# YuePanEdward/MULLS

Measured on AMD Instinct MI355X. Metric: scan-pair registrations/sec (64-beam ~120k pts, 20 ICP iters); dT vs ref, higher is better.
Workload: dtype f32

## Files before the change

mulls_amd/csrc/k_reduce.hip:

```cpp
#include "device_util.h"
#include "accum.h"
#include "solve_wave.h"

template <int LANES, int MIN_WG>
__global__ __launch_bounds__(LANES, MIN_WG) void k_accum(const uint32_t *__restrict__ leaders, const Job *__restrict__ jobs, const CloudDesc *__restrict__ descs,
														 const PairState *__restrict__ states, RunParams rp, const float4 *__restrict__ spos,
														 const float4 *__restrict__ mq, const uint8_t *__restrict__ flag, float *__restrict__ wd,
														 double *__restrict__ partial)
{
	extern __shared__ __attribute__((aligned(16))) unsigned char lds_raw[];
	__shared__ double part[MULLS_NTERM_PAD];
	const uint32_t job_idx = leaders[xcd_job(blockIdx.x, gridDim.x)];
	const Job job = jobs[job_idx];
	const PairState &ps = states[job.pair];
	if (!ps.active && !ps.want_residual)
		return;
	const CloudDesc *pd = descs + job.pair * MULLS_NC;
	const bool residual_pass = ps.want_residual != 0;
	int cnt[MULLS_NC];
	for (int c = 0; c < MULLS_NC; c++)
		cnt[c] = (int)(class_called(rp, pd[c], c) ? pd[c].valid_next : pd[c].n_valid);
	const AccumCtx A = accum_ctx(rp, job.cls, ps.iter, residual_pass, class_weight(rp, job.cls, residual_pass, cnt));
	trip_sum<true, LANES>(A, ps.x, pd[job.cls], job.start, spos, mq, flag, wd, lds_raw, part);
	if (threadIdx.x < MULLS_NTERM)
		partial[(size_t)job_idx * MULLS_NTERM + threadIdx.x] = part[threadIdx.x];
}

namespace
{
template <typename TS, int W0, int WIN, int MODE, int METRIC, int A0>
__device__ __forceinline__ void add_window(const AccumCtx &A, const double *x, const float4 P, const float4 Q, const float4 N, float wi, float &w, double *acc, const float *wpre)
{
	TS t[WIN];
#pragma unroll
	for (int k = 0; k < WIN; k++)
		t[k] = (TS)0;
	point_terms<TS, W0, WIN, MODE, METRIC>(A, x, P, Q, N, wi, w, t, wpre);
#pragma unroll
	for (int k = 0; k < WIN; k++)
		acc[W0 - A0 + k] += (double)t[k];
}
#ifndef MULLS_ACCW_WIN
#define MULLS_ACCW_WIN 9
#endif
#ifndef MULLS_ACCW_WIN_D
#define MULLS_ACCW_WIN_D 12
#endif
template <typename TS, int W0, int REM, int MODE, int METRIC, int A0>
__device__ __forceinline__ void add_windows(const AccumCtx &A, const double *x, const float4 P, const float4 Q, const float4 N, float wi, float &w, double *acc, const float *wpre)
{
	constexpr int WMAX = sizeof(TS) == 8 ? MULLS_ACCW_WIN_D : MULLS_ACCW_WIN;
	constexpr int WIN = REM < WMAX ? REM : WMAX;
	add_window<TS, W0, WIN, MODE, METRIC, A0>(A, x, P, Q, N, wi, w, acc, wpre);
	if constexpr (REM > WIN)
		add_windows<TS, W0 + WIN, REM - WIN, MODE, METRIC, A0>(A, x, P, Q, N, wi, w, acc, wpre);
}
template <typename TS, int NT, int MODE, int METRIC, int T0, int NTW>
__device__ __forceinline__ void wave_trip(const AccumCtx &A, const double *x, const CloudDesc &d, uint32_t trip0, const float4 *__restrict__ spos, const float4 *__restrict__ mq,
										   const uint8_t *__restrict__ flag, float *__restrict__ wd, double *__restrict__ out, bool owner, const LiveWord *__restrict__ live,
										   uint32_t cloud)
{
	const uint32_t lane = threadIdx.x & 63u;
	const uint32_t src_n = d.src_n, src_off = d.src_off;
	const uint32_t n_here = min(src_n - trip0, (uint32_t)MULLS_ACC_LANES), iters = (n_here + 63u) >> 6;
	const bool compacted = d.compacted != 0u;
	const uint32_t last = src_off + (compacted ? max(d.src_c, 1u) : src_n) - 1u;
	const unsigned long long below_me = (1ull << lane) - 1ull;
	static_assert(MULLS_ACC_LANES / 64 <= 64, "one LiveWord per lane covers a trip");
	uint32_t lw_lo = 0u, lw_hi = 0u, lw_below = 0u;
	if (compacted)
	{
		const LiveWord w = live[live_word_base(d, cloud) + (trip0 >> 6) + min(lane, iters - 1u)];
		lw_lo = (uint32_t)w.alive, lw_hi = (uint32_t)(w.alive >> 32), lw_below = w.below;
	}
	struct Rec
	{
		uint32_t f, g;
		bool live;
		float4 P, Q;
		float3 N;
		float w;
	};
	const bool need_w = A.residual_pass, writes_w = !A.residual_pass && (METRIC != 2 || !A.faithful);
	auto load = [&](uint32_t i) {
		Rec r;
		uint32_t g = src_off + trip0 + lane + 64u * i;
		r.live = true;
		if (compacted)
		{
			const unsigned long long alive = ((unsigned long long)(uint32_t)__builtin_amdgcn_readlane((int)lw_hi, (int)i) << 32) | (uint32_t)__builtin_amdgcn_readlane((int)lw_lo, (int)i);
			g = src_off + (uint32_t)__builtin_amdgcn_readlane((int)lw_below, (int)i) + (uint32_t)__popcll(alive & below_me);
			r.live = ((alive >> lane) & 1ull) != 0ull;
		}
		g = min(g, last);
		r.g = g;
		r.f = flag[g];
		r.P = spos[g], r.Q = mq[2u * g], r.N = *reinterpret_cast<const float3 *>(mq + 2u * g + 1u);
		r.w = need_w ? wd[g] : 0.0f;
		return r;
	};
	double acc[NTW];
#pragma unroll
	for (int k = 0; k < NTW; k++)
		acc[k] = -0.0;
#define MULLS_PIN_REC(r) asm volatile("" : "+v"((r).f), "+v"((r).P.x), "+v"((r).Q.x), "+v"((r).N.x), "+v"((r).w))
#if MULLS_ACCW_PREFETCH
	Rec cur = load(0);
#endif
	for (uint32_t i = 0; i < iters; i++)
	{
#if MULLS_ACCW_PREFETCH
		MULLS_PIN_REC(cur);
		Rec nxt = cur;
		if (i + 1u < iters)
			nxt = load(i + 1u);
#else
		Rec cur = load(i);
		MULLS_PIN_REC(cur);
#endif
		const uint32_t s = trip0 + lane + 64u * i;
		const bool valid = s < src_n && cur.live && (cur.f & (MULLS_F_ALIVE | MULLS_F_VALID)) == (MULLS_F_ALIVE | MULLS_F_VALID);
		if (valid)
		{
			float w = cur.w;
			const float4 N4 = make_float4(cur.N.x, cur.N.y, cur.N.z, 0.0f);
			const float wi = (A.inten_w && !A.residual_pass) ? point_wi(cur.P, cur.Q) : 1.0f;
			const float wpre = A.residual_pass ? 0.0f : corr_weight(A, METRIC, cur.P, cur.Q, N4, wi);
			add_windows<TS, T0, NTW, MODE, METRIC, T0>(A, x, cur.P, cur.Q, N4, wi, w, acc, A.residual_pass ? nullptr : &wpre);
			if (owner && writes_w)
				wd[cur.g] = w;
		}
#if MULLS_ACCW_PREFETCH
		cur = nxt;
#endif
	}
	if (NTW == NT && lane < MULLS_NTERM)
	{
		const bool has = MODE == 1 ? li_slot((int)lane) >= 0 : (int)lane < NT;
		if (!has)
			out[lane] = 0.0;
	}
#pragma unroll
	for (int k = 0; k < NTW; k++)
	{
		double sum = acc[k];
		sum = dpp_add_f64<0xB1>(sum);
		sum = dpp_add_f64<0x4E>(sum);
		sum = dpp_add_f64<0x141>(sum);
		sum = dpp_add_f64<0x140>(sum);
		sum = dpp_add_f64_rows<0x142, 0xa>(sum);
		sum = dpp_add_f64_rows<0x143, 0xc>(sum);
		acc[k] = sum;
	}
	if (lane == 63u)
	{
#pragma unroll
		for (int k = 0; k < NTW; k++)
			out[MODE == 1 ? li_term(T0 + k) : T0 + k] = acc[k];
	}
}
}

#ifndef MULLS_ACCW_SPLIT
#define MULLS_ACCW_SPLIT 1
#endif
#ifndef MULLS_ACCW_PREFETCH
#define MULLS_ACCW_PREFETCH 0
#endif
#ifndef MULLS_ACCW_OCC
#define MULLS_ACCW_OCC 4
#endif
#define MULLS_ACCW_WAVES 4
__global__ __launch_bounds__(64 * MULLS_ACCW_WAVES, MULLS_ACCW_OCC) void k_accum_wave(const uint32_t *__restrict__ leaders, uint32_t n_trips, const Job *__restrict__ jobs,
																					   const CloudDesc *__restrict__ descs, const PairState *__restrict__ states, RunParams rp,
																					   const float4 *__restrict__ spos, const float4 *__restrict__ mq, const uint8_t *__restrict__ flag,
																					   float *__restrict__ wd, double *__restrict__ partial)
{
	const uint32_t wave = threadIdx.x >> 6, part = wave % MULLS_ACCW_SPLIT;
	const uint32_t trip = blockIdx.x * (MULLS_ACCW_WAVES / MULLS_ACCW_SPLIT) + wave / MULLS_ACCW_SPLIT;
	if (trip >= n_trips)
		return;
	const uint32_t job_idx = leaders[trip];
	const Job job = jobs[job_idx];
	const PairState &ps = states[job.pair];
	if (!ps.active && !ps.want_residual)
		return;
	const CloudDesc *pd = descs + job.pair * MULLS_NC;
	const bool residual_pass = ps.want_residual != 0;
	int cnt[MULLS_NC];
	for (int c = 0; c < MULLS_NC; c++)
		cnt[c] = (int)(class_called(rp, pd[c], c) ? pd[c].valid_next : pd[c].n_valid);
	const AccumCtx A = accum_ctx(rp, job.cls, ps.iter, residual_pass, class_weight(rp, job.cls, residual_pass, cnt));
	const CloudDesc &d = pd[job.cls];
	const uint32_t ci = job.pair * MULLS_NC + job.cls;
	double *out = partial + (size_t)job_idx * MULLS_NTERM;
	if (d.src_n <= job.start)
	{
		if (part == 0u && (threadIdx.x & 63u) < MULLS_NTERM)
			out[threadIdx.x & 63u] = 0.0;
		return;
	}
	if (residual_pass || A.metric == 1)
	{
		if (part)
			return;
		if (!residual_pass)
			wave_trip<double, 12, 1, 1, 0, 12>(A, ps.x, d, job.start, spos, mq, flag, wd, out, true, rp.live_mask, ci);
		else if (A.metric == 0)
			wave_trip<double, 2, 0, 0, 0, 2>(A, ps.x, d, job.start, spos, mq, flag, wd, out, true, rp.live_mask, ci);
		else if (A.metric == 1)
			wave_trip<double, 2, 0, 1, 0, 2>(A, ps.x, d, job.start, spos, mq, flag, wd, out, true, rp.live_mask, ci);
		else
			wave_trip<double, 2, 0, 2, 0, 2>(A, ps.x, d, job.start, spos, mq, flag, wd, out, true, rp.live_mask, ci);
	}
#if MULLS_ACCW_SPLIT == 2
	else if (A.metric == 0)
	{
		if (part == 0u)
			wave_trip<float, 27, 0, 0, 0, 14>(A, ps.x, d, job.start, spos, mq, flag, wd, out, true, rp.live_mask, ci);
		else
			wave_trip<float, 27, 0, 0, 14, 13>(A, ps.x, d, job.start, spos, mq, flag, wd, out, false, rp.live_mask, ci);
	}
	else
	{
		if (part == 0u)
			wave_trip<float, 27, 0, 2, 0, 14>(A, ps.x, d, job.start, spos, mq, flag, wd, out, true, rp.live_mask, ci);
		else
			wave_trip<float, 27, 0, 2, 14, 13>(A, ps.x, d, job.start, spos, mq, flag, wd, out, false, rp.live_mask, ci);
	}
#else
	else if (A.metric == 0)
		wave_trip<float, 27, 0, 0, 0, 27>(A, ps.x, d, job.start, spos, mq, flag, wd, out, true, rp.live_mask, ci);
	else
		wave_trip<float, 27, 0, 2, 0, 27>(A, ps.x, d, job.start, spos, mq, flag, wd, out, true, rp.live_mask, ci);
#endif
}

namespace
{
struct FinishLds
{
	double sums[MULLS_NC][MULLS_NTERM_PAD], comb[MULLS_NTERM_PAD];
	uint32_t cnt[32];
};
__device__ __forceinline__ void finish_pair(CloudDesc *pd, const PairState &ps, const RunParams &rp, const double *__restrict__ partial,
											 PairOut &o, const uint32_t *__restrict__ pair_bbox, FinishLds *M = nullptr)
{
	if (threadIdx.x >= 192 && threadIdx.x < 198)
	{
		const uint32_t v = pair_bbox[threadIdx.x - 192];
		o.bbox[threadIdx.x - 192] = v;
		if (M)
			M->cnt[24 + threadIdx.x - 192] = v;
	}
	if (threadIdx.x < MULLS_NC * MULLS_NTERM)
	{
		const int c = threadIdx.x / MULLS_NTERM, t = threadIdx.x % MULLS_NTERM;
		if (rp.used[c])
		{
			constexpr uint32_t STEP = MULLS_ACC_LANES / MULLS_SRC_PER_BLOCK;
			double sum = 0.0;
			uint32_t j = pd[c].job_begin;
			const uint32_t je = pd[c].job_end;
			for (; j + 32u * STEP <= je; j += 32u * STEP)
			{
				double v[32];
#pragma unroll
				for (uint32_t k = 0; k < 32u; k++)
					v[k] = partial[(size_t)(j + k * STEP) * MULLS_NTERM + t];
#pragma unroll
				for (uint32_t k = 0; k < 32u; k++)
					sum += v[k];
			}
			for (; j + 16u * STEP <= je; j += 16u * STEP)
			{
				double v[16];
#pragma unroll
				for (uint32_t k = 0; k < 16u; k++)
					v[k] = partial[(size_t)(j + k * STEP) * MULLS_NTERM + t];
#pragma unroll
				for (uint32_t k = 0; k < 16u; k++)
					sum += v[k];
			}
			for (; j < je; j += STEP)
				sum += partial[(size_t)j * MULLS_NTERM + t];
			o.sums[c][t] = sum;
			if (M)
				M->sums[c][t] = sum;
		}
	}
	__syncthreads();
	if (rp.pull_comb && threadIdx.x >= 64 && threadIdx.x < 64 + MULLS_NTERM)
	{
		if (M)
		{
			combine_rows(rp, ps.want_residual != 0, M->sums, M->comb, (int)threadIdx.x - 64);
			o.comb[threadIdx.x - 64] = M->comb[threadIdx.x - 64];
		}
		else
			combine_rows(rp, ps.want_residual != 0, o.sums, o.comb, (int)threadIdx.x - 64);
	}
	if (threadIdx.x < MULLS_NC)
	{
		const int c = threadIdx.x;
		CloudDesc &d = pd[c];
		if (ps.active)
		{
			if (class_called(rp, d, c))
			{
				d.n_valid = d.valid_next;
				d.alive_cur = d.alive_next;
			}
			d.alive_next = 0;
			d.valid_next = 0;
			d.n_matched = 0;
		}
		o.n_valid[c] = d.n_valid;
		o.n_alive[c] = d.alive_cur;
		o.src_n[c] = d.src_n;
		o.tgt_n[c] = d.tgt_n;
		if (M)
			M->cnt[c] = d.n_valid, M->cnt[6 + c] = d.alive_cur, M->cnt[12 + c] = d.src_n, M->cnt[18 + c] = d.tgt_n;
	}
}
__device__ __forceinline__ void finish_pair_wave(CloudDesc *pd, const PairState &ps, const RunParams &rp, const double *__restrict__ partial, PairOut &o,
												  const uint32_t *__restrict__ pair_bbox, FinishLds &M)
{
	const uint32_t l = threadIdx.x;
	constexpr uint32_t STEP = MULLS_ACC_LANES / MULLS_SRC_PER_BLOCK;
	if (l >= 32u && l < 38u)
	{
		const uint32_t v = pair_bbox[l - 32u];
		o.bbox[l - 32u] = v;
		M.cnt[24u + l - 32u] = v;
	}
	double sum[3] = {0.0, 0.0, 0.0};
	uint32_t j[3], je[3];
	bool on[3];
#pragma unroll
	for (int u = 0; u < 3; u++)
	{
		const uint32_t idx = l + 64u * (uint32_t)u, c = idx / MULLS_NTERM;
		on[u] = idx < MULLS_NC * MULLS_NTERM && rp.used[c < MULLS_NC ? c : 0u];
		j[u] = on[u] ? pd[c].job_begin : 0u;
		je[u] = on[u] ? pd[c].job_end : 0u;
	}
	double v[3][4];
#pragma unroll
	for (int u = 0; u < 3; u++)
	{
		const uint32_t t = (l + 64u * (uint32_t)u) % MULLS_NTERM;
#pragma unroll
		for (uint32_t k = 0; k < 4u; k++)
			v[u][k] = j[u] + k * STEP < je[u] ? partial[(size_t)(j[u] + k * STEP) * MULLS_NTERM + t] : 0.0;
	}
#pragma unroll
	for (int u = 0; u < 3; u++)
	{
		const uint32_t idx = l + 64u * (uint32_t)u, c = idx / MULLS_NTERM, t = idx % MULLS_NTERM;
#pragma unroll
		for (uint32_t k = 0; k < 4u; k++)
			if (j[u] + k * STEP < je[u])
				sum[u] += v[u][k];
		for (uint32_t jj = j[u] + 4u * STEP; jj < je[u]; jj += STEP)
			sum[u] += partial[(size_t)jj * MULLS_NTERM + t];
		if (on[u])
		{
			o.sums[c][t] = sum[u];
			M.sums[c][t] = sum[u];
		}
	}
	__syncthreads();
	if (rp.pull_comb && l < MULLS_NTERM)
	{
		combine_rows(rp, ps.want_residual != 0, M.sums, M.comb, (int)l);
		o.comb[l] = M.comb[l];
	}
	if (l >= 56u && l < 56u + MULLS_NC)
	{
		const int c = (int)l - 56;
		CloudDesc &d = pd[c];
		if (ps.active)
		{
			if (class_called(rp, d, c))
			{
				d.n_valid = d.valid_next;
				d.alive_cur = d.alive_next;
			}
			d.alive_next = 0;
			d.valid_next = 0;
			d.n_matched = 0;
		}
		o.n_valid[c] = d.n_valid;
		o.n_alive[c] = d.alive_cur;
		o.src_n[c] = d.src_n;
		o.tgt_n[c] = d.tgt_n;
		M.cnt[c] = d.n_valid, M.cnt[6 + c] = d.alive_cur, M.cnt[12 + c] = d.src_n, M.cnt[18 + c] = d.tgt_n;
	}
}
}

__global__ __launch_bounds__(MULLS_BLOCK) void k_finish(CloudDesc *__restrict__ descs, const PairState *__restrict__ states, RunParams rp,
														 const double *__restrict__ partial, PairOut *__restrict__ out, const uint32_t *__restrict__ bbox,
														 uint32_t pair_base, uint4 *__restrict__ host_words, uint32_t *__restrict__ ticket,
														 volatile uint32_t *host_epoch, uint32_t epoch)
{
	const uint32_t pair = pair_base + blockIdx.x;
	const int active = states[pair].active, want_residual = states[pair].want_residual;
	if (active || want_residual)
		finish_pair(descs + pair * MULLS_NC, states[pair], rp, partial, out[pair], bbox + pair * 6);
	if (!host_words)
		return;
	__syncthreads();
	const uint32_t row_words = MULLS_NTERM_PAD / 2, head_words = 8, wpp = head_words + row_words;
	if (threadIdx.x < wpp)
	{
		const uint4 *dev = reinterpret_cast<const uint4 *>(&out[pair]);
		const uint32_t src = threadIdx.x < head_words ? (MULLS_NC + 1u) * row_words + threadIdx.x : MULLS_NC * row_words + (threadIdx.x - head_words);
		host_words[(size_t)pair * wpp + threadIdx.x] = dev[src];
	}
	__threadfence_system();
	__syncthreads();
	if (threadIdx.x == 0)
	{
		const uint32_t t = atomicAdd(ticket, 1u);
		if (t == gridDim.x - 1u)
		{
			*ticket = 0u;
			__threadfence_system();
			*host_epoch = epoch;
		}
	}
}

static_assert(sizeof(PairOut) == (MULLS_NC + 1) * MULLS_NTERM_PAD * 8 + 128, "PairOut = class rows + combined row + one 128-B counter block");
__global__ __launch_bounds__(MULLS_BLOCK) void k_pull_outs(const uint4 *__restrict__ dev_words, uint4 *__restrict__ host_words, RunParams rp,
															uint32_t pair_base, uint32_t npairs, uint32_t *__restrict__ ticket,
															volatile uint32_t *host_epoch, uint32_t epoch)
{
	const uint32_t row_words = MULLS_NTERM_PAD / 2, head_words = 8, rec_words = sizeof(PairOut) / 16;
	uint32_t n_used = 0;
	for (int c = 0; c < MULLS_NC; c++)
		n_used += rp.used[c] ? 1u : 0u;
	const uint32_t wpp = head_words + row_words * (rp.pull_comb ? 1u : n_used);
	const uint32_t i = blockIdx.x * blockDim.x + threadIdx.x;
	if (i < npairs * wpp)
	{
		const uint32_t p = pair_base + i / wpp, w = i % wpp;
		uint32_t src = (MULLS_NC + 1u) * row_words + w;
		if (w >= head_words && rp.pull_comb)
			src = MULLS_NC * row_words + (w - head_words);
		else if (w >= head_words)
		{
			uint32_t rank = (w - head_words) / row_words, cls = 0;
			for (uint32_t c = 0; c < MULLS_NC; c++)
				if (rp.used[c])
				{
					if (rank == 0)
					{
						cls = c;
						break;
					}
					rank--;
				}
			src = cls * row_words + (w - head_words) % row_words;
		}
		host_words[(size_t)p * wpp + w] = dev_words[(size_t)p * rec_words + src];
	}
	__threadfence_system();
	__syncthreads();
	if (threadIdx.x == 0)
	{
		const uint32_t t = atomicAdd(ticket, 1u);
		if (t == gridDim.x - 1u)
		{
			*ticket = 0u;
			__threadfence_system();
			*host_epoch = epoch;
		}
	}
}

__global__ __launch_bounds__(64) void k_step_init(uint32_t npairs, const PairSetup *__restrict__ setup, mulls::IcpConst K, mulls::StepState *__restrict__ steps,
												  PairState *__restrict__ states)
{
	const uint32_t pair = blockIdx.x * 64u + threadIdx.x;
	if (pair >= npairs)
		return;
	mulls::StepState &S = steps[pair];
	static_assert(sizeof(mulls::StepState) % 8 == 0, "StepState is cleared / moved in 8-byte words");
	unsigned long long *w = reinterpret_cast<unsigned long long *>(&S);
	for (uint32_t k = 0; k < sizeof(mulls::StepState) / 8; k++)
		w[k] = 0ull;
	mulls::pair_iter_init(S.h, setup[pair].guess, K);
	S.first = 1u;
	PairState &ps = states[pair];
	for (int k = 0; k < 12; k++)
		ps.T[k] = (k % 5 == 0) ? 1.0 : 0.0;
	for (int k = 0; k < 6; k++)
		ps.x[k] = 0.0;
	for (int c = 0; c < MULLS_NC; c++)
		ps.thr[c] = K.dis_thre_unit;
	ps.iter = 0;
	ps.active = S.h.active;
	ps.want_residual = 0;
	ps.pad_[0] = ps.pad_[1] = ps.pad_[2] = 0;
}

struct StepLds
{
	mulls::StepState S;
	SolveWs ws;
	double comb[MULLS_NTERM_PAD];
	uint32_t cnt[32];
	uint32_t jobs[MULLS_NC], n0[MULLS_NC];
	int go, iter, active, resid, done, left;
};
constexpr uint32_t STEP_WORDS = (uint32_t)(sizeof(mulls::StepState) / 8), STEP_WORDS_PER_LANE = (STEP_WORDS + 63u) / 64u;
__device__ __forceinline__ bool step_pair(uint32_t pair, const CloudDesc *__restrict__ descs, PairState *__restrict__ states, const RunParams &rp, const mulls::IcpConst &K,
										   const PairOut *__restrict__ out, mulls::StepState *__restrict__ steps, IcpOut *__restrict__ results, int brute, StepLds &L,
										   const unsigned long long *sw = nullptr)
{
	const int l = (int)threadIdx.x;
	const bool PRE = sw != nullptr;
	mulls::StepState &S = L.S;
	if (l == 0)
	{
		L.active = states[pair].active;
		L.resid = states[pair].want_residual;
		L.iter = states[pair].iter;
		L.left = 0;
	}
	__syncthreads();
	if (L.active || L.resid)
	{
		const PairOut &o = out[pair];
		if (l < 64)
		{
			const unsigned long long *src = reinterpret_cast<const unsigned long long *>(&steps[pair]);
			unsigned long long *dst = reinterpret_cast<unsigned long long *>(&S);
			if (PRE)
			{
#pragma unroll
				for (uint32_t k = 0; k < STEP_WORDS_PER_LANE; k++)
					if ((uint32_t)l + 64u * k < STEP_WORDS)
						dst[(uint32_t)l + 64u * k] = sw[k];
			}
			else
				for (uint32_t w = (uint32_t)l; w < STEP_WORDS; w += 64u)
					dst[w] = src[w];
		}
		if (!PRE)
		{
			if (l < MULLS_NTERM_PAD)
				L.comb[l] = o.comb[l];
			if (l < 30)
				L.cnt[l] = (&o.n_valid[0])[l];
		}
		if (l < MULLS_NC)
		{
			const CloudDesc &d = descs[pair * MULLS_NC + l];
			L.jobs[l] = d.job_end - d.job_begin;
			L.n0[l] = d.src_n0;
		}
		__syncthreads();
		const uint32_t *n_valid = L.cnt, *n_alive = L.cnt + 6, *src_n = L.cnt + 12, *tgt_n = L.cnt + 18, *obox = L.cnt + 24;
		mulls::PairIter &h = S.h;
		if (l == 0)
		{
			L.go = 0;
			if (L.resid)
				mulls::step_residual(h, K, L.comb[0], L.comb[1]);
			else
			{
				const int i = L.iter;
				h.iters = i + 1;
				if (S.first)
				{
					int sfc = 0;
					for (int c = 0; c < MULLS_NC; c++)
					{
						const uint32_t n0 = rp.undistort ? L.n0[c] : src_n[c];
						S.nsrc0[c] = n0;
						S.ntgt0[c] = tgt_n[c];
						S.alive_prev[c] = src_n[c];
						if ((c == 1 || c == 2 || c == 3) && rp.used[c])
							sfc += (int)n0;
					}
					h.src_feature_count = sfc;
					for (int k = 0; k < 6; k++)
						S.bbox[k] = obox[k];
					S.first = 0u;
				}
				for (int c = 0; c < MULLS_NC; c++)
				{
					if (rp.used[c] && S.alive_prev[c] >= 3u && tgt_n[c] >= 3u)
					{
						if (brute)
							S.pair_evals += (unsigned long long)S.alive_prev[c] * tgt_n[c];
						S.src_pts += S.alive_prev[c];
						S.tgt_pts += tgt_n[c];
						S.tgt_job_pts += (unsigned long long)tgt_n[c] * L.jobs[c];
					}
					S.alive_prev[c] = n_alive[c];
					S.ncorr[c] = n_valid[c];
					S.corr_pts += n_valid[c];
				}
				L.go = mulls::step_counts(h, K, n_valid) ? 1 : 0;
			}
		}
		__syncthreads();
		if (L.go && l < 64)
			solve_wave(h, K, L.comb, L.iter, L.ws);
		__syncthreads();
		if (l == 0)
		{
			L.done = (!h.active && !h.want_residual) ? 1 : 0;
			L.left = L.done ? 0 : 1;
			if (L.done)
				h.guess = h.temp * h.guess;
		}
		__syncthreads();
		PairState &ps = states[pair];
		if (l < 12)
			ps.T[l] = h.temp.at(l / 4, l % 4);
		else if (l < 18)
			ps.x[l - 12] = h.x[l - 12];
		else if (l < 24)
			ps.thr[l - 18] = h.thr[l - 18];
		else if (l == 24)
		{
			ps.iter = h.want_residual ? h.iters - 1 : L.iter + 1;
			ps.active = h.active ? 1 : 0;
			ps.want_residual = h.want_residual ? 1 : 0;
		}
		if (l < 64)
		{
			unsigned long long *dst = reinterpret_cast<unsigned long long *>(&steps[pair]);
			const unsigned long long *src = reinterpret_cast<const unsigned long long *>(&S);
			for (uint32_t w = (uint32_t)l; w < sizeof(mulls::StepState) / 8; w += 64u)
				dst[w] = src[w];
		}
		if (L.done)
		{
			IcpOut &O = results[pair];
			if (l < 16)
				O.T[l] = h.guess.v[l];
			if (l < 36)
				O.info[l] = h.info.v[l];
			if (l >= 40 && l < 46)
			{
				const int c = l - 40;
				O.ncorr[c] = S.ncorr[c];
				O.nsrc0[c] = S.nsrc0[c];
				O.ntgt0[c] = S.ntgt0[c];
				O.bbox[c] = S.bbox[c];
			}
			if (l == 63)
			{
				O.sigma2 = h.sigma2;
				O.ratio = h.ratio;
				O.code = h.code;
				O.iters = h.iters;
				O.singular = h.singular;
				O.trace_len = 0;
				O.src_pts = S.src_pts;
				O.tgt_pts = S.tgt_pts;
				O.corr_pts = S.corr_pts;
				O.tgt_job_pts = S.tgt_job_pts;
				O.pair_evals = S.pair_evals;
			}
		}
	}
	return L.left != 0;
}

__global__ __launch_bounds__(64) void k_step(const CloudDesc *__restrict__ descs, PairState *__restrict__ states, RunParams rp, mulls::IcpConst K,
											 const PairOut *__restrict__ out, mulls::StepState *__restrict__ steps, IcpOut *__restrict__ results, int brute,
											 uint32_t pair_base)
{
	__shared__ StepLds L;
	(void)step_pair(pair_base + blockIdx.x, descs, states, rp, K, out, steps, results, brute, L);
}

__global__ __launch_bounds__(64) void k_sum_step(CloudDesc *__restrict__ descs, PairState *__restrict__ states, RunParams rp, mulls::IcpConst K,
												 const double *__restrict__ partial, PairOut *__restrict__ out, const uint32_t *__restrict__ bbox,
												 mulls::StepState *__restrict__ steps, IcpOut *__restrict__ results, int brute, uint32_t pair_base)
{
	__shared__ StepLds L;
	__shared__ FinishLds F;
	const uint32_t pair = pair_base + blockIdx.x;
	const bool live = states[pair].active || states[pair].want_residual;
	unsigned long long sw[STEP_WORDS_PER_LANE];
	if (live)
	{
		const unsigned long long *src = reinterpret_cast<const unsigned long long *>(&steps[pair]);
#pragma unroll
		for (uint32_t k = 0; k < STEP_WORDS_PER_LANE; k++)
			sw[k] = src[min(threadIdx.x + 64u * k, STEP_WORDS - 1u)];
		finish_pair_wave(descs + pair * MULLS_NC, states[pair], rp, partial, out[pair], bbox + pair * 6, F);
	}
	__syncthreads();
	if (threadIdx.x < MULLS_NTERM_PAD)
		L.comb[threadIdx.x] = F.comb[threadIdx.x];
	if (threadIdx.x < 30u)
		L.cnt[threadIdx.x] = F.cnt[threadIdx.x];
	(void)step_pair(pair, descs, states, rp, K, out, steps, results, brute, L, sw);
}

__global__ __launch_bounds__(MULLS_BLOCK) void k_finish_step(CloudDesc *__restrict__ descs, PairState *__restrict__ states, RunParams rp, mulls::IcpConst K,
															  const double *__restrict__ partial, PairOut *__restrict__ out, const uint32_t *__restrict__ bbox,
															  mulls::StepState *__restrict__ steps, IcpOut *__restrict__ results, int brute, uint32_t *__restrict__ ticket,
															  volatile unsigned long long *host_word, uint32_t epoch, uint32_t pair_base)
{
	__shared__ StepLds L;
	const uint32_t pair = pair_base + blockIdx.x;
	const bool live = states[pair].active || states[pair].want_residual;
	unsigned long long sw[STEP_WORDS_PER_LANE];
	if (live && threadIdx.x < 64u)
	{
		const unsigned long long *src = reinterpret_cast<const unsigned long long *>(&steps[pair]);
#pragma unroll
		for (uint32_t k = 0; k < STEP_WORDS_PER_LANE; k++)
			sw[k] = src[min(threadIdx.x + 64u * k, STEP_WORDS - 1u)];
	}
	__shared__ FinishLds F;
	if (live)
		finish_pair(descs + pair * MULLS_NC, states[pair], rp, partial, out[pair], bbox + pair * 6, &F);
	__syncthreads();
	if (threadIdx.x < MULLS_NTERM_PAD)
		L.comb[threadIdx.x] = F.comb[threadIdx.x];
	else if (threadIdx.x >= 64u && threadIdx.x < 94u)
		L.cnt[threadIdx.x - 64u] = F.cnt[threadIdx.x - 64u];
	const bool left = step_pair(pair, descs, states, rp, K, out, steps, results, brute, L, sw);
	if (threadIdx.x == 0)
	{
		unsigned long long *t64 = reinterpret_cast<unsigned long long *>(ticket);
		const unsigned long long old = atomicAdd(t64, ((unsigned long long)(left ? 1u : 0u) << 32) | 1ull);
		if ((uint32_t)old == gridDim.x - 1u)
		{
			const uint32_t n_left = (uint32_t)(old >> 32) + (left ? 1u : 0u);
			*t64 = 0ull;
			__threadfence_system();
			*host_word = (unsigned long long)epoch << 32 | n_left;
		}
	}
}

__global__ __launch_bounds__(1024) void k_step_publish(const PairState *__restrict__ states, uint32_t npairs, volatile unsigned long long *host_word, uint32_t epoch)
{
	int mine = 0;
	for (uint32_t p = threadIdx.x; p < npairs; p += 1024u)
		mine += (states[p].active || states[p].want_residual) ? 1 : 0;
	__shared__ uint32_t s_left;
	if (threadIdx.x == 0)
		s_left = 0u;
	__syncthreads();
	for (int off = 32; off > 0; off >>= 1)
		mine += __shfl_down(mine, off);
	if ((threadIdx.x & 63u) == 0u && mine)
		atomicAdd(&s_left, (uint32_t)mine);
	__syncthreads();
	if (threadIdx.x == 0)
	{
		__threadfence_system();
		*host_word = (unsigned long long)epoch << 32 | s_left;
	}
}

static_assert(sizeof(PairState) % 16 == 0, "PairState must be a whole number of uint4 words");
__global__ void k_push_states(const uint4 *__restrict__ host_words, uint4 *__restrict__ dev_words, uint32_t nwords)
{
	const uint32_t i = blockIdx.x * blockDim.x + threadIdx.x;
	if (i < nwords)
		dev_words[i] = host_words[i];
}

__global__ void k_transform_aos(float4 *__restrict__ recs, uint32_t n, const double *__restrict__ T )
{
	const uint32_t i = blockIdx.x * blockDim.x + threadIdx.x;
	if (i >= n)
		return;
	float4 a = recs[(size_t)i * 3], b = recs[(size_t)i * 3 + 1];
	double x = a.x, y = a.y, z = a.z, nx = b.x, ny = b.y, nz = b.z;
	a.x = (float)(T[0] * x + T[1] * y + T[2] * z + T[3]);
	a.y = (float)(T[4] * x + T[5] * y + T[6] * z + T[7]);
	a.z = (float)(T[8] * x + T[9] * y + T[10] * z + T[11]);
	b.x = (float)(T[0] * nx + T[1] * ny + T[2] * nz);
	b.y = (float)(T[4] * nx + T[5] * ny + T[6] * nz);
	b.z = (float)(T[8] * nx + T[9] * ny + T[10] * nz);
	recs[(size_t)i * 3] = a;
	recs[(size_t)i * 3 + 1] = b;
}

__global__ void k_set_corr(uint32_t src_off, const int32_t *__restrict__ cs, const int32_t *__restrict__ ct, const float *__restrict__ cd,
						   uint32_t n, uint8_t *__restrict__ flag, int32_t *__restrict__ match, float *__restrict__ wd, uint32_t tgt_off,
						   const float4 *__restrict__ tpos, const float4 *__restrict__ tnrm, float4 *__restrict__ mq)
{
	const uint32_t i = blockIdx.x * blockDim.x + threadIdx.x;
	if (i >= n)
		return;
	const uint32_t g = src_off + (uint32_t)cs[i];
	flag[g] = MULLS_F_ALIVE | MULLS_F_VALID;
	match[g] = ct[i];
	mq[2u * g] = tpos[tgt_off + (uint32_t)ct[i]];
	mq[2u * g + 1u] = tnrm[tgt_off + (uint32_t)ct[i]];
	wd[g] = cd ? cd[i] : 0.0f;
}

#include "launch.h"

bool accum_takes_waves(const RunParams &rp, const uint32_t split[4], uint32_t wave_min_trips)
{
	const uint32_t n_trips = split[3] - split[0];
	return wave_min_trips && n_trips >= wave_min_trips && rp.faithful && rp.pull_comb;
}

void launch_accum(hipStream_t st, const BatchDev &b, const RunParams &rp, const uint32_t split[4], bool single, uint32_t wave_min_trips)
{
	(void)dev_launch<3>([](DevLaunch &) {
		return hipFuncSetAttribute(reinterpret_cast<const void *>(k_accum<1024, 2>), hipFuncAttributeMaxDynamicSharedMemorySize, (int)MULLS_RED_BYTES_HALF) == hipSuccess;
	});
	const uint32_t n_trips = split[3] - split[0];
	if (accum_takes_waves(rp, split, wave_min_trips))
	{
		hipLaunchKernelGGL(k_accum_wave, dim3((n_trips + MULLS_ACCW_WAVES / MULLS_ACCW_SPLIT - 1u) / (MULLS_ACCW_WAVES / MULLS_ACCW_SPLIT)), dim3(64 * MULLS_ACCW_WAVES), 0, st, b.ajobs + split[0], n_trips, b.jobs, b.descs, b.states, rp, b.spos,
						   b.mq, b.flag, b.wd, b.partial);
		return;
	}
	if (single)
	{
		if (split[3] > split[0])
			hipLaunchKernelGGL((k_accum<1024, 2>), dim3(split[3] - split[0]), dim3(1024), MULLS_RED_BYTES_HALF, st, b.ajobs + split[0], b.jobs, b.descs, b.states, rp, b.spos, b.mq,
							   b.flag, b.wd, b.partial);
		return;
	}
	if (split[1] > split[0])
		hipLaunchKernelGGL((k_accum<1024, 2>), dim3(split[1] - split[0]), dim3(1024), MULLS_RED_BYTES_HALF, st, b.ajobs + split[0], b.jobs, b.descs, b.states, rp, b.spos, b.mq, b.flag,
						   b.wd, b.partial);
	if (split[2] > split[1])
		hipLaunchKernelGGL((k_accum<512, 4>), dim3(split[2] - split[1]), dim3(512), MULLS_RED_BYTES_HALF / 2, st, b.ajobs + split[1], b.jobs, b.descs, b.states, rp, b.spos, b.mq, b.flag,
						   b.wd, b.partial);
	if (split[3] > split[2])
		hipLaunchKernelGGL((k_accum<256, 8>), dim3(split[3] - split[2]), dim3(256), MULLS_RED_BYTES_HALF / 4, st, b.ajobs + split[2], b.jobs, b.descs, b.states, rp, b.spos, b.mq, b.flag,
						   b.wd, b.partial);
}

void launch_finish(hipStream_t st, const BatchDev &b, const RunParams &rp, uint32_t pair_base, uint32_t npairs, uint32_t *ticket, volatile uint32_t *host_epoch, uint32_t epoch)
{
	if (!npairs)
		return;
	const bool direct = rp.pull_comb && npairs <= 64u;
	hipLaunchKernelGGL(k_finish, dim3(npairs), dim3(MULLS_BLOCK), 0, st, b.descs, b.states, rp, b.partial, b.outs, b.bbox, pair_base,
					   direct ? reinterpret_cast<uint4 *>(b.outs_pin) : nullptr, ticket, host_epoch, epoch);
	if (direct)
		return;
	uint32_t n_used = 0;
	for (int c = 0; c < MULLS_NC; c++)
		n_used += rp.used[c] ? 1u : 0u;
	const uint32_t nwords = npairs * (8u + (MULLS_NTERM_PAD / 2u) * (rp.pull_comb ? 1u : n_used));
	hipLaunchKernelGGL(k_pull_outs, dim3((nwords + MULLS_BLOCK - 1) / MULLS_BLOCK), dim3(MULLS_BLOCK), 0, st, reinterpret_cast<const uint4 *>(b.outs),
					   reinterpret_cast<uint4 *>(b.outs_pin), rp, pair_base, npairs, ticket, host_epoch, epoch);
}

void launch_step_init(hipStream_t st, const BatchDev &b, const mulls::IcpConst &K, uint32_t npairs)
{
	if (npairs)
		hipLaunchKernelGGL(k_step_init, dim3((npairs + 63u) / 64u), dim3(64), 0, st, npairs, b.setup, K, b.steps, b.states);
}

void launch_finish_step(hipStream_t st, const BatchDev &b, const RunParams &rp, const mulls::IcpConst &K, uint32_t pair_base, uint32_t npairs, unsigned long long *host_word, uint32_t epoch,
						int brute, uint32_t *ticket, bool sum_step)
{
	if (!npairs)
		return;
	if (ticket)
	{
		hipLaunchKernelGGL(k_finish_step, dim3(npairs), dim3(MULLS_BLOCK), 0, st, b.descs, b.states, rp, K, b.partial, b.outs, b.bbox, b.steps, b.icp_outs, brute, ticket, host_word, epoch,
						   pair_base);
		return;
	}
	if (sum_step && rp.pull_comb)
		hipLaunchKernelGGL(k_sum_step, dim3(npairs), dim3(64), 0, st, b.descs, b.states, rp, K, b.partial, b.outs, b.bbox, b.steps, b.icp_outs, brute, pair_base);
	else
	{
		hipLaunchKernelGGL(k_finish, dim3(npairs), dim3(MULLS_BLOCK), 0, st, b.descs, b.states, rp, b.partial, b.outs, b.bbox, pair_base, static_cast<uint4 *>(nullptr),
						   static_cast<uint32_t *>(nullptr), static_cast<volatile uint32_t *>(nullptr), 0u);
		hipLaunchKernelGGL(k_step, dim3(npairs), dim3(64), 0, st, b.descs, b.states, rp, K, b.outs, b.steps, b.icp_outs, brute, pair_base);
	}
	hipLaunchKernelGGL(k_step_publish, dim3(1), dim3(1024), 0, st, b.states + pair_base, npairs, host_word, epoch);
}

void launch_push_states(hipStream_t st, const BatchDev &b, uint32_t pair_base, uint32_t npairs)
{
	const PairState *host_states = b.states_pin + pair_base;
	PairState *dev_states = b.states + pair_base;
	const uint32_t nwords = npairs * (uint32_t)(sizeof(PairState) / 16);
	if (nwords)
		hipLaunchKernelGGL(k_push_states, dim3((nwords + 255) / 256), dim3(256), 0, st, reinterpret_cast<const uint4 *>(host_states),
						   reinterpret_cast<uint4 *>(dev_states), nwords);
}

void launch_transform_aos(hipStream_t st, float4 *recs, uint32_t n, const double *T12)
{
	if (n)
		hipLaunchKernelGGL(k_transform_aos, dim3((n + 255) / 256), dim3(256), 0, st, recs, n, T12);
}

void launch_set_corr(hipStream_t st, const BatchDev &b, uint32_t src_off, const int32_t *cs, const int32_t *ct, const float *cd, uint32_t n, uint32_t tgt_off)
{
	if (n)
		hipLaunchKernelGGL(k_set_corr, dim3((n + 255) / 256), dim3(256), 0, st, src_off, cs, ct, cd, n, b.flag, b.match, b.wd, tgt_off, b.tpos, b.tnrm, b.mq);
}
```

Baseline: 301,700.

## Stream accumulation inputs through per-wave LDS ring via global_load_lds

Replaces the per-iteration register loads in the wave accumulation loop with a per-wave LDS ring buffer (depth 2 by default), filled asynchronously with global_load_lds requests issued DEPTH-1 rounds ahead. Explicit vmcnt waits, which also account for the weight store, gate consumption of each round. The aim is to hide global memory latency without holding prefetched records in VGPRs. It adds about 13 KB of LDS per block, which may lower occupancy, and relies on fragile vmcnt bookkeeping. The old register prefetch option is removed.

```diff
diff --git a/mulls_amd/csrc/k_reduce.hip b/mulls_amd/csrc/k_reduce.hip
--- a/mulls_amd/csrc/k_reduce.hip
+++ b/mulls_amd/csrc/k_reduce.hip
@@ -1,6 +1,7 @@
 #include "device_util.h"
 #include "accum.h"
 #include "solve_wave.h"
+#include <type_traits>
 
 template <int LANES, int MIN_WG>
 __global__ __launch_bounds__(LANES, MIN_WG) void k_accum(const uint32_t *__restrict__ leaders, const Job *__restrict__ jobs, const CloudDesc *__restrict__ descs,
@@ -55,14 +56,46 @@
 	if constexpr (REM > WIN)
 		add_windows<TS, W0 + WIN, REM - WIN, MODE, METRIC, A0>(A, x, P, Q, N, wi, w, acc, wpre);
 }
+#ifndef MULLS_ACCW_RING
+#define MULLS_ACCW_RING 2
+#endif
+static_assert(MULLS_ACCW_RING == 0 || MULLS_ACCW_RING == 2 || MULLS_ACCW_RING == 3, "MULLS_ACCW_RING: 0, 2 or 3");
+struct AccwRound
+{
+	float4 P[64], Q[64], N[64];
+	uint32_t f[64];
+};
+struct AccwRoundW : AccwRound
+{
+	float w[64];
+};
+#define MULLS_ACCW_RING_BYTES (MULLS_ACCW_RING == 3 ? 3 * sizeof(AccwRound) : MULLS_ACCW_RING * sizeof(AccwRoundW))
+#define MULLS_LDS_REQUEST(SIZE, src, lds_block) \
+	__builtin_amdgcn_global_load_lds((const __attribute__((address_space(1))) void *)(src), (__attribute__((address_space(3))) void *)(lds_block), SIZE, 0, 0)
+template <int N>
+__device__ __forceinline__ void wait_vm_le()
+{
+	asm volatile("s_waitcnt vmcnt(%0)" ::"n"(N) : "memory");
+}
+template <int K>
+__device__ __forceinline__ void wait_vm_upto(uint32_t n)
+{
+	if constexpr (K == 0)
+		wait_vm_le<0>();
+	else if (n >= (uint32_t)K)
+		wait_vm_le<K>();
+	else
+		wait_vm_upto<K - 1>(n);
+}
 template <typename TS, int NT, int MODE, int METRIC, int T0, int NTW>
 __device__ __forceinline__ void wave_trip(const AccumCtx &A, const double *x, const CloudDesc &d, uint32_t trip0, const float4 *__restrict__ spos, const float4 *__restrict__ mq,
 										   const uint8_t *__restrict__ flag, float *__restrict__ wd, double *__restrict__ out, bool owner, const LiveWord *__restrict__ live,
-										   uint32_t cloud)
+										   uint32_t cloud, unsigned char *ring_mem)
 {
 	const uint32_t lane = threadIdx.x & 63u;
 	const uint32_t src_n = d.src_n, src_off = d.src_off;
-	const uint32_t n_here = min(src_n - trip0, (uint32_t)MULLS_ACC_LANES), iters = (n_here + 63u) >> 6;
+	const uint32_t n_here = min(src_n - trip0, (uint32_t)MULLS_ACC_LANES);
+	const uint32_t iters = (uint32_t)__builtin_amdgcn_readfirstlane((int)((n_here + 63u) >> 6));
 	const bool compacted = d.compacted != 0u;
 	const uint32_t last = src_off + (compacted ? max(d.src_c, 1u) : src_n) - 1u;
 	const unsigned long long below_me = (1ull << lane) - 1ull;
@@ -82,42 +115,75 @@
 		float w;
 	};
 	const bool need_w = A.residual_pass, writes_w = !A.residual_pass && (METRIC != 2 || !A.faithful);
+	auto where = [&](uint32_t i, bool &was_live) {
+		uint32_t g = src_off + trip0 + lane + 64u * i;
+		was_live = true;
+		if (compacted)
+		{
+			const unsigned long long alive = ((unsigned long long)(uint32_t)__builtin_amdgcn_readlane((int)lw_hi, (int)i) << 32) | (uint32_t)__builtin_amdgcn_readlane((int)lw_lo, (int)i);
+			g = src_off + (uint32_t)__builtin_amdgcn_readlane((int)lw_below, (int)i) + (uint32_t)__popcll(alive & below_me);
+			was_live = ((alive >> lane) & 1ull) != 0ull;
+		}
+		return min(g, last);
+	};
+#if MULLS_ACCW_RING
+	constexpr bool RING_W = NT == 2;
+	constexpr int PER_ROUND = RING_W ? 5 : 4;
+	using Round = typename std::conditional<RING_W, AccwRoundW, AccwRound>::type;
+	constexpr uint32_t DEPTH = MULLS_ACCW_RING_BYTES / sizeof(Round) < MULLS_ACCW_RING ? MULLS_ACCW_RING_BYTES / sizeof(Round) : MULLS_ACCW_RING;
+	static_assert(DEPTH >= 2 && DEPTH <= 3 && DEPTH * sizeof(Round) <= MULLS_ACCW_RING_BYTES, "the ring fits the wave's memory (at depth 1 the store counted below would be OLDER than the round's requests)");
+	Round *const ring = reinterpret_cast<Round *>(ring_mem);
+	auto request = [&](uint32_t i) {
+		bool unused;
+		const uint32_t g = where(i, unused);
+		Round &b = ring[i % DEPTH];
+		MULLS_LDS_REQUEST(16, spos + g, b.P);
+		MULLS_LDS_REQUEST(16, mq + 2u * g, b.Q);
+		MULLS_LDS_REQUEST(12, mq + 2u * g + 1u, b.N);
+		MULLS_LDS_REQUEST(1, flag + g, b.f);
+		if constexpr (RING_W)
+			MULLS_LDS_REQUEST(4, wd + g, static_cast<AccwRoundW &>(b).w);
+	};
+	uint32_t stored = 0u;
+	auto wait_round = [&](uint32_t later) { wait_vm_upto<(int)(DEPTH - 1u) * PER_ROUND + 1>(later * (uint32_t)PER_ROUND + stored); };
+	auto load = [&](uint32_t i) {
+		if (i + (DEPTH - 1u) < iters)
+			request(i + (DEPTH - 1u));
+		wait_round(min(iters - 1u - i, DEPTH - 1u));
+		Rec r;
+		r.g = where(i, r.live);
+		const Round &b = ring[i % DEPTH];
+		r.f = reinterpret_cast<const uint8_t *>(b.f)[4u * lane];
+		r.P = b.P[lane], r.Q = b.Q[lane], r.N = make_float3(b.N[lane].x, b.N[lane].y, b.N[lane].z);
+		r.w = 0.0f;
+		if constexpr (RING_W)
+			r.w = need_w ? static_cast<const AccwRoundW &>(b).w[lane] : 0.0f;
+		return r;
+	};
+#else
 	auto load = [&](uint32_t i) {
 		Rec r;
-		uint32_t g = src_off + trip0 + lane + 64u * i;
-		r.live = true;
-		if (compacted)
-		{
-			const unsigned long long alive = ((unsigned long long)(uint32_t)__builtin_amdgcn_readlane((int)lw_hi, (int)i) << 32) | (uint32_t)__builtin_amdgcn_readlane((int)lw_lo, (int)i);
-			g = src_off + (uint32_t)__builtin_amdgcn_readlane((int)lw_below, (int)i) + (uint32_t)__popcll(alive & below_me);
-			r.live = ((alive >> lane) & 1ull) != 0ull;
-		}
-		g = min(g, last);
+		const uint32_t g = where(i, r.live);
 		r.g = g;
 		r.f = flag[g];
 		r.P = spos[g], r.Q = mq[2u * g], r.N = *reinterpret_cast<const float3 *>(mq + 2u * g + 1u);
 		r.w = need_w ? wd[g] : 0.0f;
 		return r;
 	};
+#endif
 	double acc[NTW];
 #pragma unroll
 	for (int k = 0; k < NTW; k++)
 		acc[k] = -0.0;
-#define MULLS_PIN_REC(r) asm volatile("" : "+v"((r).f), "+v"((r).P.x), "+v"((r).Q.x), "+v"((r).N.x), "+v"((r).w))
-#if MULLS_ACCW_PREFETCH
-	Rec cur = load(0);
+#define MULLS_PIN_REC(r) asm volatile("" : "+v"((r).f), "+v"((r).P.x), "+v"((r).Q.x), "+v"((r).N.x), "+v"((r).N.y), "+v"((r).N.z), "+v"((r).w))
+#if MULLS_ACCW_RING
+	for (uint32_t i = 0; i + 1u < DEPTH && i < iters; i++)
+		request(i);
 #endif
 	for (uint32_t i = 0; i < iters; i++)
 	{
-#if MULLS_ACCW_PREFETCH
-		MULLS_PIN_REC(cur);
-		Rec nxt = cur;
-		if (i + 1u < iters)
-			nxt = load(i + 1u);
-#else
 		Rec cur = load(i);
 		MULLS_PIN_REC(cur);
-#endif
 		const uint32_t s = trip0 + lane + 64u * i;
 		const bool valid = s < src_n && cur.live && (cur.f & (MULLS_F_ALIVE | MULLS_F_VALID)) == (MULLS_F_ALIVE | MULLS_F_VALID);
 		if (valid)
@@ -130,8 +196,8 @@
 			if (owner && writes_w)
 				wd[cur.g] = w;
 		}
-#if MULLS_ACCW_PREFETCH
-		cur = nxt;
+#if MULLS_ACCW_RING
+		stored = (owner && writes_w && __builtin_amdgcn_ballot_w64(valid) != 0ull) ? 1u : 0u;
 #endif
 	}
 	if (NTW == NT && lane < MULLS_NTERM)
@@ -164,9 +230,6 @@
 #ifndef MULLS_ACCW_SPLIT
 #define MULLS_ACCW_SPLIT 1
 #endif
-#ifndef MULLS_ACCW_PREFETCH
-#define MULLS_ACCW_PREFETCH 0
-#endif
 #ifndef MULLS_ACCW_OCC
 #define MULLS_ACCW_OCC 4
 #endif
@@ -176,7 +239,15 @@
 																					   const float4 *__restrict__ spos, const float4 *__restrict__ mq, const uint8_t *__restrict__ flag,
 																					   float *__restrict__ wd, double *__restrict__ partial)
 {
-	const uint32_t wave = threadIdx.x >> 6, part = wave % MULLS_ACCW_SPLIT;
+#if MULLS_ACCW_RING
+	__shared__ __attribute__((aligned(16))) unsigned char rings[MULLS_ACCW_WAVES][MULLS_ACCW_RING_BYTES];
+#endif
+	const uint32_t wave = (uint32_t)__builtin_amdgcn_readfirstlane((int)(threadIdx.x >> 6)), part = wave % MULLS_ACCW_SPLIT;
+#if MULLS_ACCW_RING
+	unsigned char *const ring = rings[wave];
+#else
+	unsigned char *const ring = nullptr;
+#endif
 	const uint32_t trip = blockIdx.x * (MULLS_ACCW_WAVES / MULLS_ACCW_SPLIT) + wave / MULLS_ACCW_SPLIT;
 	if (trip >= n_trips)
 		return;
@@ -205,34 +276,34 @@
 		if (part)
 			return;
 		if (!residual_pass)
-			wave_trip<double, 12, 1, 1, 0, 12>(A, ps.x, d, job.start, spos, mq, flag, wd, out, true, rp.live_mask, ci);
+			wave_trip<double, 12, 1, 1, 0, 12>(A, ps.x, d, job.start, spos, mq, flag, wd, out, true, rp.live_mask, ci, ring);
 		else if (A.metric == 0)
-			wave_trip<double, 2, 0, 0, 0, 2>(A, ps.x, d, job.start, spos, mq, flag, wd, out, true, rp.live_mask, ci);
+			wave_trip<double, 2, 0, 0, 0, 2>(A, ps.x, d, job.start, spos, mq, flag, wd, out, true, rp.live_mask, ci, ring);
 		else if (A.metric == 1)
-			wave_trip<double, 2, 0, 1, 0, 2>(A, ps.x, d, job.start, spos, mq, flag, wd, out, true, rp.live_mask, ci);
+			wave_trip<double, 2, 0, 1, 0, 2>(A, ps.x, d, job.start, spos, mq, flag, wd, out, true, rp.live_mask, ci, ring);
 		else
-			wave_trip<double, 2, 0, 2, 0, 2>(A, ps.x, d, job.start, spos, mq, flag, wd, out, true, rp.live_mask, ci);
+			wave_trip<double, 2, 0, 2, 0, 2>(A, ps.x, d, job.start, spos, mq, flag, wd, out, true, rp.live_mask, ci, ring);
 	}
 #if MULLS_ACCW_SPLIT == 2
 	else if (A.metric == 0)
 	{
 		if (part == 0u)
-			wave_trip<float, 27, 0, 0, 0, 14>(A, ps.x, d, job.start, spos, mq, flag, wd, out, true, rp.live_mask, ci);
+			wave_trip<float, 27, 0, 0, 0, 14>(A, ps.x, d, job.start, spos, mq, flag, wd, out, true, rp.live_mask, ci, ring);
 		else
-			wave_trip<float, 27, 0, 0, 14, 13>(A, ps.x, d, job.start, spos, mq, flag, wd, out, false, rp.live_mask, ci);
+			wave_trip<float, 27, 0, 0, 14, 13>(A, ps.x, d, job.start, spos, mq, flag, wd, out, false, rp.live_mask, ci, ring);
 	}
 	else
 	{
 		if (part == 0u)
-			wave_trip<float, 27, 0, 2, 0, 14>(A, ps.x, d, job.start, spos, mq, flag, wd, out, true, rp.live_mask, ci);
+			wave_trip<float, 27, 0, 2, 0, 14>(A, ps.x, d, job.start, spos, mq, flag, wd, out, true, rp.live_mask, ci, ring);
 		else
-			wave_trip<float, 27, 0, 2, 14, 13>(A, ps.x, d, job.start, spos, mq, flag, wd, out, false, rp.live_mask, ci);
+			wave_trip<float, 27, 0, 2, 14, 13>(A, ps.x, d, job.start, spos, mq, flag, wd, out, false, rp.live_mask, ci, ring);
 	}
 #else
 	else if (A.metric == 0)
-		wave_trip<float, 27, 0, 0, 0, 27>(A, ps.x, d, job.start, spos, mq, flag, wd, out, true, rp.live_mask, ci);
+		wave_trip<float, 27, 0, 0, 0, 27>(A, ps.x, d, job.start, spos, mq, flag, wd, out, true, rp.live_mask, ci, ring);
 	else
-		wave_trip<float, 27, 0, 2, 0, 27>(A, ps.x, d, job.start, spos, mq, flag, wd, out, true, rp.live_mask, ci);
+		wave_trip<float, 27, 0, 2, 0, 27>(A, ps.x, d, job.start, spos, mq, flag, wd, out, true, rp.live_mask, ci, ring);
 #endif
 }
 
```

After: 297,400. 0.986x the previous value.
